# kivicode/TensorHive-Fixed

Measured on AMD Instinct MI355X. Metric: llama3_8b_bf16_ddp_train_tokens_per_sec, higher is better.
Workload: dtype bf16; 1 GPU; model=Llama-3-8B, global_batch=8, micro_batch=8, grad_accum=1, seq_len=4096, parallelism=dp1, optimizer=AdamW (fp32 master, fused flat kernel, clip 1.0), zero=0, attention=hip, gemm_table=True, gemm_table_kind=gemm_gfx950_t32768.csv

## Files before the change

### tensorhive_fixed_amd/ops/csrc/cross_entropy.hip

```cpp
#include "th_common.h"

__global__ __launch_bounds__(512) void ce_fwd_bwd_kernel(ushort* __restrict__ logits, long ld,
                                                         const long* __restrict__ target,
                                                         float* __restrict__ loss,
                                                         float* __restrict__ lse_out, int V,
                                                         float grad_scale, int ignore_index) {
  __shared__ float sm[16], ss[16];
  const long row = blockIdx.x;
  ushort* lr = logits + row * ld;
  const int nvec = (ld & 7) == 0 ? (V >> 3) : 0;
  float m = -INFINITY, s = 0.f;
  for (int i = threadIdx.x; i < nvec; i += blockDim.x) {
    const ushort8 x = reinterpret_cast<const ushort8*>(lr)[i];
    float vmax = -INFINITY;
    float f[8];
#pragma unroll
    for (int j = 0; j < 8; ++j) {
      f[j] = bf2f(x[j]);
      vmax = fmaxf(vmax, f[j]);
    }
    float vs = 0.f;
#pragma unroll
    for (int j = 0; j < 8; ++j) vs += __expf(f[j] - vmax);
    lse_merge(m, s, vmax, vs);
  }
  for (int i = (nvec << 3) + threadIdx.x; i < V; i += blockDim.x) lse_merge(m, s, bf2f(lr[i]), 1.f);
#pragma unroll
  for (int o = 32; o > 0; o >>= 1) {
    const float m2 = __shfl_xor(m, o, 64), s2 = __shfl_xor(s, o, 64);
    lse_merge(m, s, m2, s2);
  }
  const int lane = threadIdx.x & 63, wid = threadIdx.x >> 6;
  if (lane == 0) { sm[wid] = m; ss[wid] = s; }
  __syncthreads();
  m = sm[0]; s = ss[0];
  for (int w = 1; w < (int)(blockDim.x >> 6); ++w) lse_merge(m, s, sm[w], ss[w]);
  const float lse = m + __logf(s);
  const long tgt = target[row];
  const bool valid = tgt != ignore_index && tgt >= 0 && tgt < V;
  if (threadIdx.x == 0) {
    lse_out[row] = lse;
    loss[row] = valid ? (lse - bf2f(lr[tgt])) : 0.f;
  }
  __syncthreads();
  const float gs = valid ? grad_scale : 0.f;
  for (int i = threadIdx.x; i < nvec; i += blockDim.x) {
    const ushort8 x = reinterpret_cast<const ushort8*>(lr)[i];
    ushort8 o;
#pragma unroll
    for (int j = 0; j < 8; ++j) {
      float p = __expf(bf2f(x[j]) - lse);
      if (valid && (long)(i * 8 + j) == tgt) p -= 1.f;
      o[j] = f2bf(p * gs);
    }
    reinterpret_cast<ushort8*>(lr)[i] = o;
  }
  for (int i = (nvec << 3) + threadIdx.x; i < V; i += blockDim.x) {
    float p = __expf(bf2f(lr[i]) - lse);
    if (valid && (long)i == tgt) p -= 1.f;
    lr[i] = f2bf(p * gs);
  }
}

extern "C" int th_ce_fwd_bwd(void* logits, long ld, const long* target, float* loss, float* lse,
                             long rows, int V, float grad_scale, int ignore_index, hipStream_t s) {
  if (rows <= 0 || V <= 0 || ld < V) return -1;
  ce_fwd_bwd_kernel<<<(unsigned)rows, 512, 0, s>>>((ushort*)logits, ld, target, loss, lse, V,
                                                  grad_scale, ignore_index);
  TH_CHECK_LAUNCH();
}
```

### tensorhive_fixed_amd/ops/csrc/rmsnorm.hip

```cpp
#include "th_common.h"

template <int MAXV, bool ADD>
__global__ __launch_bounds__(256) void rmsnorm_fwd_kernel(const ushort* __restrict__ x,
                                                              const ushort* __restrict__ addend,
                                                              ushort* __restrict__ xsum,
                                                              const ushort* __restrict__ w,
                                                              ushort* __restrict__ y,
                                                              float* __restrict__ rstd_out, int D,
                                                              float eps) {
  __shared__ float red[16];
  const int row = blockIdx.x;
  const int nvec = D >> 3;
  const ushort8* xr = reinterpret_cast<const ushort8*>(x + (size_t)row * D);
  ushort8 cache[MAXV];
  float ss = 0.f;
#pragma unroll
  for (int i = 0; i < MAXV; ++i) {
    const int v = threadIdx.x + i * blockDim.x;
    if (v < nvec) {
      cache[i] = xr[v];
      if (ADD) {
        const ushort8 a = reinterpret_cast<const ushort8*>(addend + (size_t)row * D)[v];
#pragma unroll
        for (int j = 0; j < 8; ++j) cache[i][j] = f2bf(bf2f(cache[i][j]) + bf2f(a[j]));
        reinterpret_cast<ushort8*>(xsum + (size_t)row * D)[v] = cache[i];
      }
#pragma unroll
      for (int j = 0; j < 8; ++j) {
        const float f = bf2f(cache[i][j]);
        ss += f * f;
      }
    }
  }
  ss = block_sum(ss, red);
  const float r = rsqrtf(ss / (float)D + eps);
  if (threadIdx.x == 0) rstd_out[row] = r;
  const ushort8* wr = reinterpret_cast<const ushort8*>(w);
  ushort8* yr = reinterpret_cast<ushort8*>(y + (size_t)row * D);
#pragma unroll
  for (int i = 0; i < MAXV; ++i) {
    const int v = threadIdx.x + i * blockDim.x;
    if (v < nvec) {
      const ushort8 wv = wr[v];
      ushort8 o;
#pragma unroll
      for (int j = 0; j < 8; ++j) o[j] = f2bf(bf2f(cache[i][j]) * r * bf2f(wv[j]));
      yr[v] = o;
    }
  }
}

template <int MAXV>
__global__ __launch_bounds__(256) void rmsnorm_bwd_kernel(const ushort* __restrict__ dy,
                                                          const ushort* __restrict__ x,
                                                          const ushort* __restrict__ w,
                                                          const float* __restrict__ rstd,
                                                          ushort* __restrict__ dx,
                                                          float* __restrict__ ws, int T, int D,
                                                          const ushort* __restrict__ dres) {
  __shared__ float red[16];
  const int nvec = D >> 3;
  float dwacc[MAXV][8];
  float wreg[MAXV][8];
  const ushort8* wr = reinterpret_cast<const ushort8*>(w);
#pragma unroll
  for (int i = 0; i < MAXV; ++i) {
    const int v = threadIdx.x + i * blockDim.x;
    ushort8 wv = (v < nvec) ? wr[v] : ushort8(0);
#pragma unroll
    for (int j = 0; j < 8; ++j) {
      dwacc[i][j] = 0.f;
      wreg[i][j] = bf2f(wv[j]);
    }
  }
  for (int row = blockIdx.x; row < T; row += gridDim.x) {
    const ushort8* xr = reinterpret_cast<const ushort8*>(x + (size_t)row * D);
    const ushort8* gr = reinterpret_cast<const ushort8*>(dy + (size_t)row * D);
    ushort8 xc[MAXV], gc[MAXV], rc[MAXV];
    float dot = 0.f;
#pragma unroll
    for (int i = 0; i < MAXV; ++i) {
      const int v = threadIdx.x + i * blockDim.x;
      if (v < nvec) {
        xc[i] = xr[v];
        gc[i] = gr[v];
        rc[i] = dres ? reinterpret_cast<const ushort8*>(dres + (size_t)row * D)[v] : ushort8(0);
#pragma unroll
        for (int j = 0; j < 8; ++j) dot += bf2f(gc[i][j]) * wreg[i][j] * bf2f(xc[i][j]);
      }
    }
    dot = block_sum(dot, red);
    const float r = rstd[row];
    const float c = dot * r * r * r / (float)D;
    ushort8* dxr = reinterpret_cast<ushort8*>(dx + (size_t)row * D);
#pragma unroll
    for (int i = 0; i < MAXV; ++i) {
      const int v = threadIdx.x + i * blockDim.x;
      if (v < nvec) {
        ushort8 o;
#pragma unroll
        for (int j = 0; j < 8; ++j) {
          const float xf = bf2f(xc[i][j]), gf = bf2f(gc[i][j]);
          o[j] = f2bf(r * gf * wreg[i][j] - xf * c + bf2f(rc[i][j]));
          dwacc[i][j] += gf * xf * r;
        }
        dxr[v] = o;
      }
    }
  }
  float* wsr = ws + (size_t)blockIdx.x * D;
#pragma unroll
  for (int i = 0; i < MAXV; ++i) {
    const int v = threadIdx.x + i * blockDim.x;
    if (v < nvec) {
      float4v* p = reinterpret_cast<float4v*>(wsr + v * 8);
      p[0] = float4v{dwacc[i][0], dwacc[i][1], dwacc[i][2], dwacc[i][3]};
      p[1] = float4v{dwacc[i][4], dwacc[i][5], dwacc[i][6], dwacc[i][7]};
    }
  }
}

__global__ __launch_bounds__(256) void slab_reduce_bf16_kernel(const float* __restrict__ ws, ushort* __restrict__ out,
                                                               int nslab, int D, int accumulate) {
  __shared__ float4v part[16][16];
  const int cg = threadIdx.x & 15, sg = threadIdx.x >> 4;
  const int c = blockIdx.x * 64 + cg * 4;
  float4v acc = {0.f, 0.f, 0.f, 0.f};
  if (c < D) {
#pragma unroll 4
    for (int b = sg; b < nslab; b += 16) acc += *reinterpret_cast<const float4v*>(ws + (size_t)b * D + c);
  }
  part[sg][cg] = acc;
  __syncthreads();
  if (sg == 0 && c < D) {
    float4v t = part[0][cg];
#pragma unroll
    for (int k = 1; k < 16; ++k) t += part[k][cg];
#pragma unroll
    for (int j = 0; j < 4; ++j) {
      float v = t[j];
      if (accumulate) v += bf2f(out[c + j]);
      out[c + j] = f2bf(v);
    }
  }
}

static int pick_maxv(int D, int threads) { return (D / 8 + threads - 1) / threads; }

extern "C" int th_rmsnorm_fwd(const void* x, const void* w, void* y, float* rstd, int T, int D,
                              float eps, hipStream_t s) {
  if (D % 8 != 0 || T <= 0) return -1;
  const int mv = pick_maxv(D, 256);
  dim3 g(T), b(256);
  if (mv <= 2)
    rmsnorm_fwd_kernel<2, false><<<g, b, 0, s>>>((const ushort*)x, nullptr, nullptr, (const ushort*)w, (ushort*)y, rstd, D, eps);
  else if (mv <= 4)
    rmsnorm_fwd_kernel<4, false><<<g, b, 0, s>>>((const ushort*)x, nullptr, nullptr, (const ushort*)w, (ushort*)y, rstd, D, eps);
  else if (mv <= 8)
    rmsnorm_fwd_kernel<8, false><<<g, b, 0, s>>>((const ushort*)x, nullptr, nullptr, (const ushort*)w, (ushort*)y, rstd, D, eps);
  else
    return -2;
  TH_CHECK_LAUNCH();
}

extern "C" int th_rmsnorm_add_fwd(const void* x, const void* addend, const void* w, void* xsum, void* y,
                                  float* rstd, int T, int D, float eps, hipStream_t s) {
  if (D % 8 != 0 || T <= 0) return -1;
  const int mv = pick_maxv(D, 256);
  dim3 g(T), b(256);
#define TH_RMS_ADD(MV)                                                                                   \
  rmsnorm_fwd_kernel<MV, true><<<g, b, 0, s>>>((const ushort*)x, (const ushort*)addend, (ushort*)xsum, \
                                               (const ushort*)w, (ushort*)y, rstd, D, eps)
  if (mv <= 2)
    TH_RMS_ADD(2);
  else if (mv <= 4)
    TH_RMS_ADD(4);
  else if (mv <= 8)
    TH_RMS_ADD(8);
  else
    return -2;
#undef TH_RMS_ADD
  TH_CHECK_LAUNCH();
}

extern "C" int th_rmsnorm_bwd(const void* dy, const void* x, const void* w, const float* rstd,
                              void* dx, void* dw, float* ws, int nblk, int T, int D,
                              int accumulate, const void* dres, hipStream_t s) {
  if (D % 8 != 0 || T <= 0 || nblk <= 0) return -1;
  const int mv = pick_maxv(D, 256);
  dim3 g(nblk), b(256);
  if (mv <= 2)
    rmsnorm_bwd_kernel<2><<<g, b, 0, s>>>((const ushort*)dy, (const ushort*)x, (const ushort*)w, rstd, (ushort*)dx, ws, T, D, (const ushort*)dres);
  else if (mv <= 4)
    rmsnorm_bwd_kernel<4><<<g, b, 0, s>>>((const ushort*)dy, (const ushort*)x, (const ushort*)w, rstd, (ushort*)dx, ws, T, D, (const ushort*)dres);
  else if (mv <= 8)
    rmsnorm_bwd_kernel<8><<<g, b, 0, s>>>((const ushort*)dy, (const ushort*)x, (const ushort*)w, rstd, (ushort*)dx, ws, T, D, (const ushort*)dres);
  else
    return -2;
  slab_reduce_bf16_kernel<<<dim3((D + 63) / 64), dim3(256), 0, s>>>(ws, (ushort*)dw, nblk, D, accumulate);
  TH_CHECK_LAUNCH();
}
```

### tensorhive_fixed_amd/ops/csrc/swiglu.hip

```cpp
#include "th_common.h"

__device__ __forceinline__ float sigmoidf_(float g) { return 1.f / (1.f + __expf(-g)); }

__global__ __launch_bounds__(256) void swiglu_fwd_kernel(const ushort* __restrict__ gu,
                                                         ushort* __restrict__ out, long T, int F) {
  const int cpr = F >> 3;
  for (long row = blockIdx.x; row < T; row += gridDim.x) {
    const ushort* g_row = gu + row * 2 * F;
    ushort* o_row = out + row * F;
    for (int c = threadIdx.x; c < cpr; c += blockDim.x) {
      const ushort8 g = *reinterpret_cast<const ushort8*>(g_row + c * 8);
      const ushort8 u = *reinterpret_cast<const ushort8*>(g_row + F + c * 8);
      ushort8 o;
#pragma unroll
      for (int j = 0; j < 8; ++j) {
        const float gf = bf2f(g[j]);
        o[j] = f2bf(gf * sigmoidf_(gf) * bf2f(u[j]));
      }
      *reinterpret_cast<ushort8*>(o_row + c * 8) = o;
    }
  }
}

__global__ __launch_bounds__(256) void swiglu_bwd_kernel(const ushort* __restrict__ dout,
                                                         const ushort* __restrict__ gu,
                                                         ushort* __restrict__ dgu, long T, int F) {
  const int cpr = F >> 3;
  for (long row = blockIdx.x; row < T; row += gridDim.x) {
    for (int c = threadIdx.x; c < cpr; c += blockDim.x) {
      const ushort8 g = *reinterpret_cast<const ushort8*>(gu + row * 2 * F + c * 8);
      const ushort8 u = *reinterpret_cast<const ushort8*>(gu + row * 2 * F + F + c * 8);
      const ushort8 d = *reinterpret_cast<const ushort8*>(dout + row * F + c * 8);
      ushort8 dg, du;
#pragma unroll
      for (int j = 0; j < 8; ++j) {
        const float gf = bf2f(g[j]), uf = bf2f(u[j]), df = bf2f(d[j]);
        const float sg = sigmoidf_(gf);
        const float silu = gf * sg;
        du[j] = f2bf(df * silu);
        dg[j] = f2bf(df * uf * sg * (1.f + gf * (1.f - sg)));
      }
      *reinterpret_cast<ushort8*>(dgu + row * 2 * F + c * 8) = dg;
      *reinterpret_cast<ushort8*>(dgu + row * 2 * F + F + c * 8) = du;
    }
  }
}

constexpr int ST_R = 128, ST_C = 64;

__device__ __forceinline__ int st_swz(int r) { return 2 * (((r >> 1) & 1) | (((r >> 3) & 1) << 1)); }
__device__ __forceinline__ int st_off(int r, int chunk) { return r * 128 + ((chunk ^ st_swz(r)) << 4); }

typedef short i16x4s __attribute__((ext_vector_type(4)));
#define ST_LDS __attribute__((address_space(3)))

__global__ __launch_bounds__(256) void swiglu_bwd_t_kernel(const ushort* __restrict__ dout,
                                                           const ushort* __restrict__ gu,
                                                           ushort* __restrict__ dgu,
                                                           ushort* __restrict__ dguT, long T, int F) {
  __shared__ __attribute__((aligned(16))) char tile[2 * ST_R * 128];
  const int tid = threadIdx.x;
  const long ntc = F / ST_C;
  const long r0 = (blockIdx.x / ntc) * ST_R, c0 = (blockIdx.x % ntc) * ST_C;
  const int lch = tid & 7, lc = lch * 8;
  ushort8 g[4], u[4], d[4];
#pragma unroll
  for (int i = 0; i < 4; ++i) {
    const long row = r0 + (tid >> 3) + 32 * i;
    const long rr = row < T ? row : T - 1;
    g[i] = *reinterpret_cast<const ushort8*>(gu + rr * 2 * F + c0 + lc);
    u[i] = *reinterpret_cast<const ushort8*>(gu + rr * 2 * F + F + c0 + lc);
    d[i] = *reinterpret_cast<const ushort8*>(dout + rr * F + c0 + lc);
  }
#pragma unroll
  for (int i = 0; i < 4; ++i) {
    const int lr = (tid >> 3) + 32 * i;
    const long row = r0 + lr;
    ushort8 dg, du;
#pragma unroll
    for (int j = 0; j < 8; ++j) {
      const float gf = bf2f(g[i][j]), uf = bf2f(u[i][j]), df = bf2f(d[i][j]);
      const float sg = sigmoidf_(gf);
      du[j] = f2bf(df * gf * sg);
      dg[j] = f2bf(df * uf * sg * (1.f + gf * (1.f - sg)));
    }
    if (row < T) {
      *reinterpret_cast<ushort8*>(dgu + row * 2 * F + c0 + lc) = dg;
      *reinterpret_cast<ushort8*>(dgu + row * 2 * F + F + c0 + lc) = du;
    }
    *reinterpret_cast<ushort8*>(tile + st_off(lr, lch)) = dg;
    *reinterpret_cast<ushort8*>(tile + ST_R * 128 + st_off(lr, lch)) = du;
  }
  __syncthreads();
  const int lane = tid & 63, w = tid >> 6, grp = lane >> 4, i16 = lane & 15, q = i16 >> 2, p = i16 & 3;
#pragma unroll
  for (int k = 0; k < 8; ++k) {
    const int step = w * 8 + k;
    const int half = step >> 4, fb = (step >> 2) & 3, tg0 = (step & 3) * 32;
    const int rbase = tg0 + 8 * grp;
    const int col = fb * 16 + 4 * p;
    const char* base = tile + half * ST_R * 128 + ((col & 7) << 1);
    const int ch = col >> 3;
    const i16x4s lo = __builtin_amdgcn_ds_read_tr16_b64_v4i16((ST_LDS i16x4s*)(base + st_off(rbase + q, ch)));
    const i16x4s hi = __builtin_amdgcn_ds_read_tr16_b64_v4i16((ST_LDS i16x4s*)(base + st_off(rbase + 4 + q, ch)));
    ushort8 o;
#pragma unroll
    for (int e = 0; e < 4; ++e) {
      o[e] = (ushort)lo[e];
      o[4 + e] = (ushort)hi[e];
    }
    const long feat = (long)half * F + c0 + fb * 16 + i16;
    const long tok = r0 + rbase;
    if (tok < T) *reinterpret_cast<ushort8*>(dguT + feat * T + tok) = o;
  }
}

static unsigned grid_for(long rows) {
  long g = rows;
  if (g > 4096) g = 4096;
  if (g < 1) g = 1;
  return (unsigned)g;
}

extern "C" int th_swiglu_fwd(const void* gu, void* out, long T, int F, hipStream_t s) {
  if (F % 8 != 0 || T <= 0) return -1;
  swiglu_fwd_kernel<<<grid_for(T), 256, 0, s>>>((const ushort*)gu, (ushort*)out, T, F);
  TH_CHECK_LAUNCH();
}

extern "C" int th_swiglu_bwd(const void* dout, const void* gu, void* dgu, long T, int F,
                             hipStream_t s) {
  if (F % 8 != 0 || T <= 0) return -1;
  swiglu_bwd_kernel<<<grid_for(T), 256, 0, s>>>((const ushort*)dout, (const ushort*)gu,
                                                          (ushort*)dgu, T, F);
  TH_CHECK_LAUNCH();
}

extern "C" int th_swiglu_bwd_t(const void* dout, const void* gu, void* dgu, void* dguT, long T, int F,
                               hipStream_t s) {
  if (F % ST_C != 0 || T <= 0 || T % 8 != 0) return -1;
  const long tiles = ((T + ST_R - 1) / ST_R) * (F / ST_C);
  if (tiles > 0x7fffffffL) return -2;
  swiglu_bwd_t_kernel<<<(unsigned)tiles, 256, 0, s>>>((const ushort*)dout, (const ushort*)gu, (ushort*)dgu,
                                                      (ushort*)dguT, T, F);
  TH_CHECK_LAUNCH();
}
```

### tensorhive_fixed_amd/ops/csrc/transpose.hip

```cpp
#include "th_common.h"

template <int TR, int TC>
__global__ __launch_bounds__(256) void transpose_bf16_kernel(const ushort* __restrict__ in,
                                                             ushort* __restrict__ out, long R, long C,
                                                             long ld_in) {
  constexpr int PITCH = TC + 2;
  constexpr int LPR = TC / 8;
  constexpr int RPP = 256 / LPR;
  constexpr int OPL = 256 / TC;
  constexpr int RPL = TR / OPL;
  __shared__ ushort tile[TR * PITCH];
  const int tid = threadIdx.x;
  const long ntc = (C + TC - 1) / TC;
  const long bt = blockIdx.x;
  const long r0 = (bt / ntc) * TR, c0 = (bt % ntc) * TC;

  const int lc = (tid % LPR) * 8;
  ushort8 v[TR / RPP];
#pragma unroll
  for (int i = 0; i < TR / RPP; ++i) {
    const int lr = tid / LPR + RPP * i;
    v[i] = ushort8(0);
    if (r0 + lr < R && c0 + lc < C) v[i] = *reinterpret_cast<const ushort8*>(in + (r0 + lr) * ld_in + c0 + lc);
  }
#pragma unroll
  for (int i = 0; i < TR / RPP; ++i) {
    const int lr = tid / LPR + RPP * i;
    unsigned* dst = reinterpret_cast<unsigned*>(tile + lr * PITCH + lc);
#pragma unroll
    for (int j = 0; j < 4; ++j) dst[j] = (unsigned)v[i][2 * j] | ((unsigned)v[i][2 * j + 1] << 16);
  }
  __syncthreads();

  const int oc = tid / OPL;
  const int orr = (tid % OPL) * RPL;
  if (c0 + oc >= C) return;
  ushort* orow = out + (c0 + oc) * R + r0 + orr;
#pragma unroll
  for (int q = 0; q < RPL / 8; ++q) {
    ushort8 w;
#pragma unroll
    for (int j = 0; j < 8; ++j) w[j] = tile[(orr + 8 * q + j) * PITCH + oc];
    if (r0 + orr + 8 * q < R) *reinterpret_cast<ushort8*>(orow + 8 * q) = w;
  }
}

extern "C" int th_transpose_bf16(const void* in, void* out, long R, long C, long ld_in, int tile, hipStream_t s) {
  if (R <= 0 || C <= 0 || R % 8 || C % 8 || ld_in % 8 || ld_in < C) return -1;
  auto launch = [&](auto kern, long tr, long tc) {
    const long tiles = ((R + tr - 1) / tr) * ((C + tc - 1) / tc);
    if (tiles > 0x7fffffffL) return -2;
    kern<<<(unsigned)tiles, 256, 0, s>>>((const ushort*)in, (ushort*)out, R, C, ld_in);
    return (int)hipGetLastError();
  };
  if (tile == 0) tile = C > 16384 ? 1 : 3;
  switch (tile) {
    case 2: return launch(transpose_bf16_kernel<128, 128>, 128, 128);
    case 3: return launch(transpose_bf16_kernel<64, 128>, 64, 128);
    default: return launch(transpose_bf16_kernel<128, 64>, 128, 64);
  }
}
```

Baseline: 27200 tokens/s.

## Rework cross-entropy, rmsnorm bwd, swiglu and transpose kernels for bandwidth

Cross-entropy for large vocabularies now holds the logits row in registers, so the backward pass skips a second global read. The rmsnorm backward prefetches the next row while computing the current one. SwiGLU uses an exp2/rcp sigmoid with Newton refinement and processes two vectors per iteration. Transpose becomes a persistent, double-buffered kernel using swizzled LDS and ds_read_tr16 transposed reads, with new default tile choices. Together these trade extra register and LDS pressure, plus a small numerical change in sigmoid, for lower memory traffic in elementwise and transpose kernels.

Measured after the change: 27250 tokens/s (median of 6 runs). Within noise of the previous version (+0.2%).

```diff
diff --git a/tensorhive_fixed_amd/ops/csrc/cross_entropy.hip b/tensorhive_fixed_amd/ops/csrc/cross_entropy.hip
--- a/tensorhive_fixed_amd/ops/csrc/cross_entropy.hip
+++ b/tensorhive_fixed_amd/ops/csrc/cross_entropy.hip
@@ -1,4 +1,86 @@
 #include "th_common.h"
+
+__device__ __forceinline__ void ce_block_merge(float& m, float& s, float* sm, float* ss) {
+#pragma unroll
+  for (int o = 32; o > 0; o >>= 1) {
+    const float m2 = __shfl_xor(m, o, 64), s2 = __shfl_xor(s, o, 64);
+    lse_merge(m, s, m2, s2);
+  }
+  const int lane = threadIdx.x & 63, wid = threadIdx.x >> 6;
+  if (lane == 0) { sm[wid] = m; ss[wid] = s; }
+  __syncthreads();
+  m = sm[0]; s = ss[0];
+  for (int w = 1; w < (int)((blockDim.x + 63) >> 6); ++w) lse_merge(m, s, sm[w], ss[w]);
+}
+
+__device__ __forceinline__ void ce_vec_lse(const ushort8 x, float& m, float& s) {
+  float vmax = -INFINITY;
+  float f[8];
+#pragma unroll
+  for (int j = 0; j < 8; ++j) {
+    f[j] = bf2f(x[j]);
+    vmax = fmaxf(vmax, f[j]);
+  }
+  float vs = 0.f;
+#pragma unroll
+  for (int j = 0; j < 8; ++j) vs += __expf(f[j] - vmax);
+  lse_merge(m, s, vmax, vs);
+}
+
+__device__ __forceinline__ ushort8 ce_vec_grad(const ushort8 x, int col0, float lse, bool valid, long tgt,
+                                               float gs) {
+  ushort8 o;
+#pragma unroll
+  for (int j = 0; j < 8; ++j) {
+    float p = __expf(bf2f(x[j]) - lse);
+    if (valid && (long)(col0 + j) == tgt) p -= 1.f;
+    o[j] = f2bf(p * gs);
+  }
+  return o;
+}
+
+template <int NV>
+__global__ __launch_bounds__(1024) void ce_fwd_bwd_regs_kernel(ushort* __restrict__ logits, long ld,
+                                                              const long* __restrict__ target,
+                                                              float* __restrict__ loss,
+                                                              float* __restrict__ lse_out, int V,
+                                                              float grad_scale, int ignore_index) {
+  __shared__ float sm[16], ss[16];
+  const long row = blockIdx.x;
+  ushort* lr = logits + row * ld;
+  const int nvec = V >> 3;
+  ushort8 cache[NV];
+#pragma unroll
+  for (int k = 0; k < NV; ++k) {
+    const int i = threadIdx.x + k * blockDim.x;
+    cache[k] = reinterpret_cast<const ushort8*>(lr)[i < nvec ? i : nvec - 1];
+  }
+  float m = -INFINITY, s = 0.f;
+#pragma unroll
+  for (int k = 0; k < NV; ++k)
+    if ((int)(threadIdx.x + k * blockDim.x) < nvec) ce_vec_lse(cache[k], m, s);
+  for (int i = (nvec << 3) + threadIdx.x; i < V; i += blockDim.x) lse_merge(m, s, bf2f(lr[i]), 1.f);
+  ce_block_merge(m, s, sm, ss);
+  const float lse = m + __logf(s);
+  const long tgt = target[row];
+  const bool valid = tgt != ignore_index && tgt >= 0 && tgt < V;
+  if (threadIdx.x == 0) {
+    lse_out[row] = lse;
+    loss[row] = valid ? (lse - bf2f(lr[tgt])) : 0.f;
+  }
+  __syncthreads();
+  const float gs = valid ? grad_scale : 0.f;
+#pragma unroll
+  for (int k = 0; k < NV; ++k) {
+    const int i = threadIdx.x + k * blockDim.x;
+    if (i < nvec) reinterpret_cast<ushort8*>(lr)[i] = ce_vec_grad(cache[k], i * 8, lse, valid, tgt, gs);
+  }
+  for (int i = (nvec << 3) + threadIdx.x; i < V; i += blockDim.x) {
+    float p = __expf(bf2f(lr[i]) - lse);
+    if (valid && (long)i == tgt) p -= 1.f;
+    lr[i] = f2bf(p * gs);
+  }
+}
 
 __global__ __launch_bounds__(512) void ce_fwd_bwd_kernel(ushort* __restrict__ logits, long ld,
                                                          const long* __restrict__ target,
@@ -62,10 +144,19 @@
   }
 }
 
+constexpr int CE_REG_MIN_V = 16384;
+constexpr int CE_REG_MAX_V = 131072;
+
 extern "C" int th_ce_fwd_bwd(void* logits, long ld, const long* target, float* loss, float* lse,
                              long rows, int V, float grad_scale, int ignore_index, hipStream_t s) {
   if (rows <= 0 || V <= 0 || ld < V) return -1;
-  ce_fwd_bwd_kernel<<<(unsigned)rows, 512, 0, s>>>((ushort*)logits, ld, target, loss, lse, V,
-                                                  grad_scale, ignore_index);
+  if (V > CE_REG_MIN_V && V <= CE_REG_MAX_V && (ld & 7) == 0) {
+    const unsigned threads = (V >> 3) <= 512 * 16 ? 512 : 1024;
+    ce_fwd_bwd_regs_kernel<16><<<(unsigned)rows, threads, 0, s>>>((ushort*)logits, ld, target, loss, lse, V,
+                                                                 grad_scale, ignore_index);
+  } else {
+    ce_fwd_bwd_kernel<<<(unsigned)rows, 512, 0, s>>>((ushort*)logits, ld, target, loss, lse, V, grad_scale,
+                                                    ignore_index);
+  }
   TH_CHECK_LAUNCH();
 }
diff --git a/tensorhive_fixed_amd/ops/csrc/rmsnorm.hip b/tensorhive_fixed_amd/ops/csrc/rmsnorm.hip
--- a/tensorhive_fixed_amd/ops/csrc/rmsnorm.hip
+++ b/tensorhive_fixed_amd/ops/csrc/rmsnorm.hip
@@ -73,18 +73,29 @@
       wreg[i][j] = bf2f(wv[j]);
     }
   }
-  for (int row = blockIdx.x; row < T; row += gridDim.x) {
+  ushort8 xc[MAXV], gc[MAXV], rc[MAXV];
+  auto load_row = [&](int row, ushort8* xo, ushort8* go, ushort8* ro) {
     const ushort8* xr = reinterpret_cast<const ushort8*>(x + (size_t)row * D);
     const ushort8* gr = reinterpret_cast<const ushort8*>(dy + (size_t)row * D);
-    ushort8 xc[MAXV], gc[MAXV], rc[MAXV];
-    float dot = 0.f;
 #pragma unroll
     for (int i = 0; i < MAXV; ++i) {
       const int v = threadIdx.x + i * blockDim.x;
       if (v < nvec) {
-        xc[i] = xr[v];
-        gc[i] = gr[v];
-        rc[i] = dres ? reinterpret_cast<const ushort8*>(dres + (size_t)row * D)[v] : ushort8(0);
+        xo[i] = xr[v];
+        go[i] = gr[v];
+        ro[i] = dres ? reinterpret_cast<const ushort8*>(dres + (size_t)row * D)[v] : ushort8(0);
+      }
+    }
+  };
+  if ((int)blockIdx.x < T) load_row(blockIdx.x, xc, gc, rc);
+  for (int row = blockIdx.x; row < T; row += gridDim.x) {
+    ushort8 xn[MAXV], gn[MAXV], rn[MAXV];
+    if (row + (int)gridDim.x < T) load_row(row + gridDim.x, xn, gn, rn);
+    float dot = 0.f;
+#pragma unroll
+    for (int i = 0; i < MAXV; ++i) {
+      const int v = threadIdx.x + i * blockDim.x;
+      if (v < nvec) {
 #pragma unroll
         for (int j = 0; j < 8; ++j) dot += bf2f(gc[i][j]) * wreg[i][j] * bf2f(xc[i][j]);
       }
@@ -106,6 +117,12 @@
         }
         dxr[v] = o;
       }
+    }
+#pragma unroll
+    for (int i = 0; i < MAXV; ++i) {
+      xc[i] = xn[i];
+      gc[i] = gn[i];
+      rc[i] = rn[i];
     }
   }
   float* wsr = ws + (size_t)blockIdx.x * D;
diff --git a/tensorhive_fixed_amd/ops/csrc/swiglu.hip b/tensorhive_fixed_amd/ops/csrc/swiglu.hip
--- a/tensorhive_fixed_amd/ops/csrc/swiglu.hip
+++ b/tensorhive_fixed_amd/ops/csrc/swiglu.hip
@@ -1,47 +1,88 @@
 #include "th_common.h"
 
-__device__ __forceinline__ float sigmoidf_(float g) { return 1.f / (1.f + __expf(-g)); }
+constexpr float SG_INV = 0.0625f;
 
-__global__ __launch_bounds__(256) void swiglu_fwd_kernel(const ushort* __restrict__ gu,
-                                                         ushort* __restrict__ out, long T, int F) {
-  const int cpr = F >> 3;
-  for (long row = blockIdx.x; row < T; row += gridDim.x) {
-    const ushort* g_row = gu + row * 2 * F;
-    ushort* o_row = out + row * F;
-    for (int c = threadIdx.x; c < cpr; c += blockDim.x) {
-      const ushort8 g = *reinterpret_cast<const ushort8*>(g_row + c * 8);
-      const ushort8 u = *reinterpret_cast<const ushort8*>(g_row + F + c * 8);
-      ushort8 o;
+__device__ __forceinline__ float sigmoidf_(float g) {
+#pragma clang fp contract(off)
+  const float e = __builtin_amdgcn_exp2f(g * -1.4426950408889634f);
+  const float d = fminf(fmaf(e, SG_INV, SG_INV), 3.402823466e+38f);
+  float r = __builtin_amdgcn_rcpf(d);
+  r = fmaf(fmaf(-d, r, 1.f), r, r);
+  float q = r;
+  q = fmaf(fmaf(-d, q, 1.f), r, q);
+  q = fmaf(fmaf(-d, q, 1.f), r, q);
+  return q * SG_INV;
+}
+
+__device__ __forceinline__ ushort8 swiglu_fwd8(const ushort8 g, const ushort8 u) {
+  ushort8 o;
 #pragma unroll
-      for (int j = 0; j < 8; ++j) {
-        const float gf = bf2f(g[j]);
-        o[j] = f2bf(gf * sigmoidf_(gf) * bf2f(u[j]));
-      }
-      *reinterpret_cast<ushort8*>(o_row + c * 8) = o;
-    }
+  for (int j = 0; j < 8; ++j) {
+    const float gf = bf2f(g[j]);
+    o[j] = f2bf(gf * sigmoidf_(gf) * bf2f(u[j]));
+  }
+  return o;
+}
+
+__device__ __forceinline__ void swiglu_bwd8(const ushort8 g, const ushort8 u, const ushort8 d, ushort8& dg,
+                                            ushort8& du) {
+#pragma unroll
+  for (int j = 0; j < 8; ++j) {
+    const float gf = bf2f(g[j]), uf = bf2f(u[j]), df = bf2f(d[j]);
+    const float sg = sigmoidf_(gf);
+    const float silu = gf * sg;
+    du[j] = f2bf(df * silu);
+    dg[j] = f2bf(df * uf * sg * (1.f + gf * (1.f - sg)));
   }
 }
 
-__global__ __launch_bounds__(256) void swiglu_bwd_kernel(const ushort* __restrict__ dout,
-                                                         const ushort* __restrict__ gu,
-                                                         ushort* __restrict__ dgu, long T, int F) {
+constexpr int SW_THREADS = 256;
+
+__global__ __launch_bounds__(SW_THREADS) void swiglu_fwd_kernel(const ushort* __restrict__ gu,
+                                                                ushort* __restrict__ out, long T, int F) {
   const int cpr = F >> 3;
   for (long row = blockIdx.x; row < T; row += gridDim.x) {
-    for (int c = threadIdx.x; c < cpr; c += blockDim.x) {
-      const ushort8 g = *reinterpret_cast<const ushort8*>(gu + row * 2 * F + c * 8);
-      const ushort8 u = *reinterpret_cast<const ushort8*>(gu + row * 2 * F + F + c * 8);
-      const ushort8 d = *reinterpret_cast<const ushort8*>(dout + row * F + c * 8);
+    const ushort8* g_row = reinterpret_cast<const ushort8*>(gu + row * 2 * F);
+    const ushort8* u_row = reinterpret_cast<const ushort8*>(gu + row * 2 * F + F);
+    ushort8* o_row = reinterpret_cast<ushort8*>(out + row * F);
+    int c = threadIdx.x;
+    for (; c + SW_THREADS < cpr; c += 2 * SW_THREADS) {
+      const ushort8 g0 = g_row[c], u0 = u_row[c];
+      const ushort8 g1 = g_row[c + SW_THREADS], u1 = u_row[c + SW_THREADS];
+      o_row[c] = swiglu_fwd8(g0, u0);
+      o_row[c + SW_THREADS] = swiglu_fwd8(g1, u1);
+    }
+    if (c < cpr) o_row[c] = swiglu_fwd8(g_row[c], u_row[c]);
+  }
+}
+
+__global__ __launch_bounds__(SW_THREADS) void swiglu_bwd_kernel(const ushort* __restrict__ dout,
+                                                                const ushort* __restrict__ gu,
+                                                                ushort* __restrict__ dgu, long T, int F) {
+  const int cpr = F >> 3;
+  for (long row = blockIdx.x; row < T; row += gridDim.x) {
+    const ushort8* g_row = reinterpret_cast<const ushort8*>(gu + row * 2 * F);
+    const ushort8* u_row = reinterpret_cast<const ushort8*>(gu + row * 2 * F + F);
+    const ushort8* d_row = reinterpret_cast<const ushort8*>(dout + row * F);
+    ushort8* dg_row = reinterpret_cast<ushort8*>(dgu + row * 2 * F);
+    ushort8* du_row = reinterpret_cast<ushort8*>(dgu + row * 2 * F + F);
+    int c = threadIdx.x;
+    for (; c + SW_THREADS < cpr; c += 2 * SW_THREADS) {
+      const ushort8 g0 = g_row[c], u0 = u_row[c], d0 = d_row[c];
+      const ushort8 g1 = g_row[c + SW_THREADS], u1 = u_row[c + SW_THREADS], d1 = d_row[c + SW_THREADS];
+      ushort8 dg0, du0, dg1, du1;
+      swiglu_bwd8(g0, u0, d0, dg0, du0);
+      swiglu_bwd8(g1, u1, d1, dg1, du1);
+      dg_row[c] = dg0;
+      du_row[c] = du0;
+      dg_row[c + SW_THREADS] = dg1;
+      du_row[c + SW_THREADS] = du1;
+    }
+    if (c < cpr) {
       ushort8 dg, du;
-#pragma unroll
-      for (int j = 0; j < 8; ++j) {
-        const float gf = bf2f(g[j]), uf = bf2f(u[j]), df = bf2f(d[j]);
-        const float sg = sigmoidf_(gf);
-        const float silu = gf * sg;
-        du[j] = f2bf(df * silu);
-        dg[j] = f2bf(df * uf * sg * (1.f + gf * (1.f - sg)));
-      }
-      *reinterpret_cast<ushort8*>(dgu + row * 2 * F + c * 8) = dg;
-      *reinterpret_cast<ushort8*>(dgu + row * 2 * F + F + c * 8) = du;
+      swiglu_bwd8(g_row[c], u_row[c], d_row[c], dg, du);
+      dg_row[c] = dg;
+      du_row[c] = du;
     }
   }
 }
@@ -77,13 +118,7 @@
     const int lr = (tid >> 3) + 32 * i;
     const long row = r0 + lr;
     ushort8 dg, du;
-#pragma unroll
-    for (int j = 0; j < 8; ++j) {
-      const float gf = bf2f(g[i][j]), uf = bf2f(u[i][j]), df = bf2f(d[i][j]);
-      const float sg = sigmoidf_(gf);
-      du[j] = f2bf(df * gf * sg);
-      dg[j] = f2bf(df * uf * sg * (1.f + gf * (1.f - sg)));
-    }
+    swiglu_bwd8(g[i], u[i], d[i], dg, du);
     if (row < T) {
       *reinterpret_cast<ushort8*>(dgu + row * 2 * F + c0 + lc) = dg;
       *reinterpret_cast<ushort8*>(dgu + row * 2 * F + F + c0 + lc) = du;
@@ -124,14 +159,14 @@
 
 extern "C" int th_swiglu_fwd(const void* gu, void* out, long T, int F, hipStream_t s) {
   if (F % 8 != 0 || T <= 0) return -1;
-  swiglu_fwd_kernel<<<grid_for(T), 256, 0, s>>>((const ushort*)gu, (ushort*)out, T, F);
+  swiglu_fwd_kernel<<<grid_for(T), SW_THREADS, 0, s>>>((const ushort*)gu, (ushort*)out, T, F);
   TH_CHECK_LAUNCH();
 }
 
 extern "C" int th_swiglu_bwd(const void* dout, const void* gu, void* dgu, long T, int F,
                              hipStream_t s) {
   if (F % 8 != 0 || T <= 0) return -1;
-  swiglu_bwd_kernel<<<grid_for(T), 256, 0, s>>>((const ushort*)dout, (const ushort*)gu,
+  swiglu_bwd_kernel<<<grid_for(T), SW_THREADS, 0, s>>>((const ushort*)dout, (const ushort*)gu,
                                                           (ushort*)dgu, T, F);
   TH_CHECK_LAUNCH();
 }
diff --git a/tensorhive_fixed_amd/ops/csrc/transpose.hip b/tensorhive_fixed_amd/ops/csrc/transpose.hip
--- a/tensorhive_fixed_amd/ops/csrc/transpose.hip
+++ b/tensorhive_fixed_amd/ops/csrc/transpose.hip
@@ -1,62 +1,99 @@
 #include "th_common.h"
+
+typedef short tp_i16x4 __attribute__((ext_vector_type(4)));
+#define TP_LDS __attribute__((address_space(3)))
+
+__device__ __forceinline__ int tp_swz(int r) { return 2 * (((r >> 1) & 1) | (((r >> 3) & 1) << 1)); }
+__device__ __forceinline__ int tp_off(int r, int chunk) { return r * 128 + ((chunk ^ tp_swz(r)) << 4); }
 
 template <int TR, int TC>
 __global__ __launch_bounds__(256) void transpose_bf16_kernel(const ushort* __restrict__ in,
                                                              ushort* __restrict__ out, long R, long C,
-                                                             long ld_in) {
-  constexpr int PITCH = TC + 2;
-  constexpr int LPR = TC / 8;
-  constexpr int RPP = 256 / LPR;
-  constexpr int OPL = 256 / TC;
-  constexpr int RPL = TR / OPL;
-  __shared__ ushort tile[TR * PITCH];
+                                                             long ld_in, int ntr, int ntc, int gq, int gr) {
+  constexpr int NP = TC / 64;
+  constexpr int PANEL = TR * 128;
+  constexpr int NV = TR * TC / 8 / 256;
+  constexpr int TG = TR / 32;
+  constexpr int SPW = NP * 4 * TG / 4;
+  static_assert(TR % 32 == 0 && TC % 64 == 0 && NV >= 1 && SPW >= 1, "tile shape");
+  __shared__ __attribute__((aligned(16))) char lds[2][NP * PANEL];
   const int tid = threadIdx.x;
-  const long ntc = (C + TC - 1) / TC;
-  const long bt = blockIdx.x;
-  const long r0 = (bt / ntc) * TR, c0 = (bt % ntc) * TC;
+  const int lane = tid & 63, w = tid >> 6, grp = lane >> 4, i16 = lane & 15, q = i16 >> 2, pp = i16 & 3;
 
-  const int lc = (tid % LPR) * 8;
-  ushort8 v[TR / RPP];
+  ushort8 v[NV];
+  auto load_tile = [&](int tr, int tc) {
+    const long r0 = (long)tr * TR, c0 = (long)tc * TC;
 #pragma unroll
-  for (int i = 0; i < TR / RPP; ++i) {
-    const int lr = tid / LPR + RPP * i;
-    v[i] = ushort8(0);
-    if (r0 + lr < R && c0 + lc < C) v[i] = *reinterpret_cast<const ushort8*>(in + (r0 + lr) * ld_in + c0 + lc);
-  }
+    for (int i = 0; i < NV; ++i) {
+      const int idx = tid + 256 * i;
+      const long row = r0 + (idx >> 3) % TR, col = c0 + (idx / (8 * TR)) * 64 + (idx & 7) * 8;
+      v[i] = ushort8(0);
+      if (row < R && col < C) v[i] = *reinterpret_cast<const ushort8*>(in + row * ld_in + col);
+    }
+  };
+
+  int tr = blockIdx.x / ntc, tc = blockIdx.x % ntc;
+  auto advance = [&](int& r, int& c) {
+    r += gq;
+    c += gr;
+    if (c >= ntc) {
+      c -= ntc;
+      ++r;
+    }
+  };
+  if (tr < ntr) load_tile(tr, tc);
+  for (int b = 0; tr < ntr; b ^= 1) {
+    const long r0 = (long)tr * TR, c0 = (long)tc * TC;
 #pragma unroll
-  for (int i = 0; i < TR / RPP; ++i) {
-    const int lr = tid / LPR + RPP * i;
-    unsigned* dst = reinterpret_cast<unsigned*>(tile + lr * PITCH + lc);
+    for (int i = 0; i < NV; ++i) {
+      const int idx = tid + 256 * i;
+      *reinterpret_cast<ushort8*>(lds[b] + (idx / (8 * TR)) * PANEL + tp_off((idx >> 3) % TR, idx & 7)) = v[i];
+    }
+    advance(tr, tc);
+    if (tr < ntr) load_tile(tr, tc);
+    __syncthreads();
+    ushort8 o[SPW];
 #pragma unroll
-    for (int j = 0; j < 4; ++j) dst[j] = (unsigned)v[i][2 * j] | ((unsigned)v[i][2 * j + 1] << 16);
-  }
-  __syncthreads();
-
-  const int oc = tid / OPL;
-  const int orr = (tid % OPL) * RPL;
-  if (c0 + oc >= C) return;
-  ushort* orow = out + (c0 + oc) * R + r0 + orr;
+    for (int k = 0; k < SPW; ++k) {
+      const int step = w * SPW + k;
+      const int tg = step % TG, fb = (step / TG) & 3, p = step / (4 * TG);
+      const int rbase = tg * 32 + 8 * grp;
+      const int col = fb * 16 + 4 * pp;
+      const char* base = lds[b] + p * PANEL + ((col & 7) << 1);
+      const int ch = col >> 3;
+      const tp_i16x4 lo = __builtin_amdgcn_ds_read_tr16_b64_v4i16((TP_LDS tp_i16x4*)(base + tp_off(rbase + q, ch)));
+      const tp_i16x4 hi = __builtin_amdgcn_ds_read_tr16_b64_v4i16((TP_LDS tp_i16x4*)(base + tp_off(rbase + 4 + q, ch)));
 #pragma unroll
-  for (int q = 0; q < RPL / 8; ++q) {
-    ushort8 w;
+      for (int e = 0; e < 4; ++e) {
+        o[k][e] = (ushort)lo[e];
+        o[k][4 + e] = (ushort)hi[e];
+      }
+    }
 #pragma unroll
-    for (int j = 0; j < 8; ++j) w[j] = tile[(orr + 8 * q + j) * PITCH + oc];
-    if (r0 + orr + 8 * q < R) *reinterpret_cast<ushort8*>(orow + 8 * q) = w;
+    for (int k = 0; k < SPW; ++k) {
+      const int step = w * SPW + k;
+      const int tg = step % TG, fb = (step / TG) & 3, p = step / (4 * TG);
+      const long oc = c0 + p * 64 + fb * 16 + i16;
+      const long orr = r0 + tg * 32 + 8 * grp;
+      if (oc < C && orr < R) *reinterpret_cast<ushort8*>(out + oc * R + orr) = o[k];
+    }
   }
 }
 
 extern "C" int th_transpose_bf16(const void* in, void* out, long R, long C, long ld_in, int tile, hipStream_t s) {
   if (R <= 0 || C <= 0 || R % 8 || C % 8 || ld_in % 8 || ld_in < C) return -1;
-  auto launch = [&](auto kern, long tr, long tc) {
-    const long tiles = ((R + tr - 1) / tr) * ((C + tc - 1) / tc);
+  auto launch = [&](auto kern, long tr, long tc, long wgs) {
+    const long ntr = (R + tr - 1) / tr, ntc = (C + tc - 1) / tc, tiles = ntr * ntc;
     if (tiles > 0x7fffffffL) return -2;
-    kern<<<(unsigned)tiles, 256, 0, s>>>((const ushort*)in, (ushort*)out, R, C, ld_in);
+    const long grid = tiles < 256 * wgs ? tiles : 256 * wgs;
+    kern<<<(unsigned)grid, 256, 0, s>>>((const ushort*)in, (ushort*)out, R, C, ld_in, (int)ntr, (int)ntc,
+                                        (int)(grid / ntc), (int)(grid % ntc));
     return (int)hipGetLastError();
   };
-  if (tile == 0) tile = C > 16384 ? 1 : 3;
+  if (tile == 0) tile = R * C >= (1L << 26) ? 2 : 1;
   switch (tile) {
-    case 2: return launch(transpose_bf16_kernel<128, 128>, 128, 128);
-    case 3: return launch(transpose_bf16_kernel<64, 128>, 64, 128);
-    default: return launch(transpose_bf16_kernel<128, 64>, 128, 64);
+    case 2: return launch(transpose_bf16_kernel<128, 128>, 128, 128, 2);
+    case 3: return launch(transpose_bf16_kernel<64, 128>, 64, 128, 4);
+    default: return launch(transpose_bf16_kernel<128, 64>, 128, 64, 4);
   }
 }
```
